# k2kobayashi/crank

Measured on AMD Instinct MI355X. Metric: train frames/sec, higher is better.
Workload: dtype bf16; 1 GPU; vqvae trainer step (all sub-updates), VCC2020-shaped synthetic 80-dim mlfb, 64 utterances x 500 frames per GPU, 14 speakers; trainer=vqvae, global_batch=64, batch_len=500, parallelism=dp1

## Files before the change

### crank_amd/_lib.py

```python
import ctypes
import os
from .config import cfg
from ctypes import c_char_p, c_double, c_float, c_int, c_longlong, c_ulonglong, c_void_p

_HERE = os.path.dirname(os.path.abspath(__file__))
LIB_PATH = cfg.lib_path or os.path.join(_HERE, "libcrank_hip.so")
_lib = None

ERRORS = {1: "invalid argument", 2: "HIP runtime error", 3: "unsupported shape/configuration"}


class NetDesc(ctypes.Structure):
    _fields_ = [
        ("kind", c_int), ("in_ch", c_int), ("out_ch", c_int), ("kernel_size", c_int), ("layers", c_int),
        ("stacks", c_int), ("res_ch", c_int), ("gate_ch", c_int), ("skip_ch", c_int), ("aux_ch", c_int),
        ("conv_ch", c_int), ("causal", c_int), ("use_bias", c_int), ("slope", c_float), ("dropout", c_float),
    ]


COLLATE_MAX_STREAMS = 8


class CollateStream(ctypes.Structure):
    _fields_ = [("src", c_void_p), ("ld", c_int), ("col0", c_int), ("ncols", c_int), ("dst", c_void_p)]


class CollateDesc(ctypes.Structure):
    _fields_ = [
        ("n_streams", c_int), ("streams", CollateStream * COLLATE_MAX_STREAMS), ("utt_start", c_void_p),
        ("utt_spk", c_void_p), ("n_utt", c_int), ("n_spk", c_int), ("lcf0_raw", c_void_p),
        ("spk_lcf0_mean", c_void_p), ("spk_lcf0_std", c_void_p), ("raw", c_void_p), ("raw_start", c_void_p),
        ("fftl", c_int), ("hop", c_int),
    ]


ADAM_MAX_BLOCKS = 4


class AdamBlock(ctypes.Structure):
    _fields_ = [("params", c_void_p), ("grads", c_void_p), ("exp_avg", c_void_p), ("exp_avg_sq", c_void_p),
                ("n", c_longlong), ("lr_dev", c_void_p), ("step_dev", c_void_p)]


class StreamDesc(ctypes.Structure):
    _fields_ = [
        ("n_stacks", c_int), ("in_ch", c_int), ("out_ch", c_int), ("emb_dim", c_int * 3), ("emb_size", c_int * 3),
        ("cb_off", c_longlong * 3), ("enc_base", c_longlong * 3), ("dec_base", c_longlong * 3), ("causal", c_int),
        ("enc_f0", c_int), ("dec_f0", c_int), ("spk_dim", c_int), ("spk_onehot", c_int), ("n_spk", c_int),
        ("spk_off", c_longlong),
    ]


class F0StreamRound(ctypes.Structure):
    _fields_ = [("ids", c_void_p), ("utt", c_void_p), ("range", c_void_p), ("chan_bf", c_void_p), ("chan", c_void_p),
                ("n_ready", c_int), ("total_samples", c_longlong), ("total_channels", c_longlong),
                ("total_frames", c_longlong), ("total_events", c_longlong)]


P, I, LL, ULL, F, D = c_void_p, c_int, c_longlong, c_ulonglong, c_float, c_double

SIGNATURES = {
    "crk_net_create": (P, [ctypes.POINTER(NetDesc)]),
    "crk_net_destroy": (None, [P]),
    "crk_net_param_count": (LL, [P]),
    "crk_net_conv_count": (I, [P]),
    "crk_net_conv_info": (I, [P, I, ctypes.POINTER(c_longlong)]),
    "crk_net_saved_bytes": (LL, [P, I, I]),
    "crk_net_reserve": (I, [P, I, I]),
    "crk_net_scratch_bytes": (LL, [P, I, I]),
    "crk_debug_alloc_count": (LL, []),
    "crk_debug_net_paths": (I, [P, I, I]),
    "crk_debug_net_partials": (LL, [P, I, I, P, LL, P]),
    "crk_seed_next": (I, [P, P, P]),
    "crk_nets_wnorm_bwd": (I, [I, P, P]),
    "crk_nets_prepare": (I, [I, P, P, ULL, P, P]),
    "crk_nets_prepare_models": (I, [I, P, P, P, I, P, P]),
    "crk_net_forward": (I, [P, P, ULL, P, I, P, I, P, I, P, I, I, I, ULL, P]),
    "crk_net_backward": (I, [P, P, ULL, P, P, I, P, I, P, I, P, I, F, P, I, P, I, I, I, ULL, P]),
    "crk_net_backward_scaled": (I, [P, P, ULL, P, P, I, P, I, P, I, P, I, F, P, I, P, I, I, I, ULL, P, P, P]),
    "crk_net_embed_grad_supported": (I, [P, I, I, I]),
    "crk_net_backward_embed": (I, [P, P, ULL, P, P, I, P, I, P, I, P, I, F, P, I, I, I, ULL, P, LL, I, I, I, P, P]),
    "crk_vq_forward": (I, [P, I, P, I, I, I, P, P, I, P, I, P]),
    "crk_vq_forward_fused": (I, [P, I, P, I, P, I, P, I, I, I, P, P, I, P, I, P, P, P, P, P]),
    "crk_vq_image_bytes": (LL, [I, I]),
    "crk_vq_image_build_multi": (I, [I, P, P, I, P, P]),
    "crk_vq_ema_scratch_bytes": (LL, [I, I, I]),
    "crk_vq_ema_stats": (I, [P, I, P, I, I, I, P, P, P, P]),
    "crk_vq_ema_apply": (I, [P, P, P, P, P, I, I, D, D, P]),
    "crk_vq_ema_partial": (I, [P, I, P, I, I, I, P, P]),
    "crk_vq_ema_reduce_multi": (I, [I, P, P, P, P, P, P, P]),
    "crk_vq_ema_apply_multi": (I, [I, P, P, P, P, P, P, P, D, D, P]),
    "crk_vq_ema_partial_multi": (I, [I, P, P, P, P, P, P, P, P]),
    "crk_vq_ema_reduce_size_multi": (I, [I, P, P, P, P, P, P, P, D, D, P]),
    "crk_vq_ema_blend_multi": (I, [I, P, P, P, P, P, P, D, P]),
    "crk_vq_ema_blend_image_multi": (I, [I, P, P, P, P, P, P, D, P, P]),
    "crk_stft_loss_multi_fwd": (I, [P, I, P, I, I, I, I, I, P, P, P, P, F, P, P, P]),
    "crk_stft_loss_multi_fwd_grad": (I, [P, I, P, I, I, I, I, I, P, P, P, P, F, P, P, I, P, P]),
    "crk_stft_loss_multi_bwd": (I, [P, I, P, I, I, I, I, I, P, P, P, P, F, P, P, I, P]),
    "crk_loss_scratch_floats": (I, []),
    "crk_masked_loss_fwd": (I, [P, I, P, I, F, P, LL, I, I, P, P, P]),
    "crk_masked_loss_bwd": (I, [P, I, P, I, F, P, LL, I, I, P, P, P, I, P, I, P]),
    "crk_masked_loss_both_fwd": (I, [P, I, P, I, P, LL, I, P, P, P]),
    "crk_weighted_sum": (I, [I, P, P, F, P, P]),
    "crk_weighted_sum_bwd": (I, [I, P, P, P, P]),
    "crk_recon_supported": (I, [I, I, P, P, P]),
    "crk_stft_twiddle_floats": (LL, [I, I]),
    "crk_stft_twiddles": (I, [I, I, P, P, P]),
    "crk_recon_grad_floats": (LL, [I, I, I, I, P, P]),
    "crk_recon_loss_fwd": (I, [P, I, P, I, P, I, I, I, I, P, P, P, P, F, P, P, P, P]),
    "crk_recon_loss_bwd": (I, [P, I, P, I, P, I, I, I, I, P, P, P, P, P, P, P, P, P, I, P]),
    "crk_masked_loss_bwd_acc": (I, [P, I, P, I, F, P, LL, I, I, P, P, P, I, P, I, P, I, P, P]),
    "crk_vq_commit_bwd": (I, [P, I, P, I, P, LL, I, P, P, P, I, P, I, P, I, P, I, P, I, P]),
    "crk_ce_fwd": (I, [P, I, P, LL, I, I, P, P, P, P]),
    "crk_ce_bwd": (I, [P, LL, I, P, P, P, P]),
    "crk_stft_loss_fwd": (I, [P, I, P, I, I, I, I, I, I, I, P, F, F, I, P, P, P]),
    "crk_stft_loss_bwd": (I, [P, I, P, I, I, I, I, I, I, I, P, F, F, P, P, I, P]),
    "crk_adam_step": (I, [P, P, P, P, LL, P, P, F, F, F, I, P]),
    "crk_adam_step_multi": (I, [I, ctypes.POINTER(AdamBlock), F, F, F, I, P]),
    "crk_radam_step": (I, [P, P, P, P, LL, P, P, D, D, D, I, P]),
    "crk_lamb_step": (I, [P, P, P, P, P, P, I, P, I, P, P, P, P, D, D, D, I, P]),
    "crk_lamb_tile": (I, []),
    "crk_concat_embed": (I, [P, I, I, P, I, I, P, I, P, LL, P, I, P]),
    "crk_embed_bwd_scratch_floats": (LL, [LL, I, I]),
    "crk_embed_bwd": (I, [P, I, I, I, P, LL, I, P, P, P]),
    "crk_concat_embed_run": (I, [P, I, I, P, I, I, P, I, P, LL, LL, P, I, P]),
# ... 154 lines not shown
```

### crank_amd/csrc/conv_kernels.h

```cpp
#pragma once
#include <vector>

#include "runtime.h"

#define CRK_TM 128

enum { MODE_PLAIN = 0, MODE_RESFWD = 1, MODE_BWDA = 2 };

struct ConvP {
  const float* xa; int lda; int cinA; float scaleA;
  const float* xb; int ldb; int cinB; float scaleB;
  int act_in; float slope;
  float drop_p; unsigned long long drop_seed;
  const unsigned long long* drop_seed_ptr;
  int cin, cin_pad;
  const float* xc; int ldc; int cinC; int cinC_pad;
  const uint16_t* w_hi; const uint16_t* w_lo;
  const uint16_t* wc_hi; const uint16_t* wc_lo;
  const uint16_t* w2_hi; const uint16_t* w2_lo;
  const float* bias; const float* bias2a; const float* bias2b;
  int cout, cout_pad, ktaps, dil, off0;
  int B, T, tiles_per_utt;
  float* y; int ldy; int accumulate; int act_out; float out_scale;
  const float* dmask; int ldm; int dmask_act;
// ... 164 lines not shown
  int rec;
  int dbg;
};
struct StackWLayer {
  long long pt_conv, pb_conv, pt_os, pb_os, pt_aux;
  int dil, off0;
};
struct StackWP {
  const uint16_t *xb_hi, *xb_lo, *zb_hi, *zb_lo, *cb_hi, *cb_lo;
  const uint16_t *gb_hi, *gb_lo, *dxb_hi, *dxb_lo, *dsb_hi, *dsb_lo;
  const StackWLayer* layers;
  float* partials;
  int B, T, L, ktaps, aux_ch, aux_pad, cpg, G;
  int rec_g;
  float* usums; int nseg;
};
int stack_wgrad_supported(int ktaps, int max_dil, int aux_ch);
int launch_stack_wgrad(const StackWP& p, bool precise, hipStream_t s);
struct CondEmbedP {
  const float* usums; int nseg, cpg;
  const uint16_t *whi, *wlo;
  const StackBLayer* layers;
  const long long* idx; long long run;
  int B, T, L, c0, E, n_rows;
  float* dtable;
};
int launch_cond_embed_bwd(const CondEmbedP& p, hipStream_t s);
int stack_bwd_plan(StackBP& p, bool precise);
int stack2_bwd_plan(StackBP& p);
int launch_stack2_bwd(const StackBP& p, hipStream_t s);
int stack_bwd_waves(bool precise);
int launch_stack_bwd(const StackBP& p, bool precise, hipStream_t s);
int stack_fwd_plan(StackP& p, bool precise);
int launch_stack_fwd(const StackP& p, bool precise, hipStream_t s);
int stack2_fwd_plan(StackP& p);
int launch_stack2_fwd(const StackP& p, hipStream_t s);
int stack2x_fwd_plan(StackP& p);
int launch_stack2x_fwd(const StackP& p, hipStream_t s);
void conv_fill_lds(ConvP& p, int mode, bool precise);
int launch_conv(const ConvP& p, int mode, bool precise, hipStream_t s);
int wgrad_expand(const WgradP& job, bool precise, std::vector<WgradP>& out);
int launch_wgrad_table(const WgradP* d_jobs, const std::vector<WgradP>& h_jobs, int B, int T, int max_groups, bool precise,
                       hipStream_t s);
#define CRK_MAX_NETS 8
struct NetRef {
  const ConvEntry* ents; const float* params; float* grads; const float* partials; float* norms;
  uint16_t *whi, *wlo;
  int n_ents, first;
};
#define CRK_MAX_BUMPS 4
struct NetRefs { NetRef r[CRK_MAX_NETS]; int n; float* bump[CRK_MAX_BUMPS]; int n_bump; };
int launch_weight_prep_multi(const NetRefs& R, int total_entries, int nmax, hipStream_t s);
int launch_step_bump(float* const* steps, int n, hipStream_t s);
int launch_wnorm_bwd_multi(const NetRefs& R, int total_entries, hipStream_t s);
int launch_weight_prep(const ConvEntry* d_entries, int n_entries, int nmax, const float* params, uint16_t* wprep_hi,
                       uint16_t* wprep_lo, float* norms, hipStream_t s);
int launch_wnorm_bwd(const ConvEntry* d_entries, int n_entries, const float* params, float* grads,
                     const float* partials, const float* norms, hipStream_t s);
int conv_kernels_init();
```

### crank_amd/csrc/conv_kernels.hip

```cpp
#include "conv_kernels.h"

__device__ __forceinline__ int cd_row(int r, int half) { return (r & 3) + 8 * (r >> 2) + 4 * half; }

__device__ __forceinline__ float load_src(const ConvP& p, long n, int c) {
  float v;
  if (c < p.cinA) {
    v = p.xa ? p.xa[n * p.lda + c] * p.scaleA : 0.f;
  } else {
    v = p.xb ? p.xb[n * p.ldb + (c - p.cinA)] * p.scaleB : 0.f;
  }
  v = apply_act(v, p.act_in, p.slope);
  if (p.drop_p > 0.f) v *= dropout_scale(crk_seed(p.drop_seed, p.drop_seed_ptr), (unsigned long long)n * p.cin + c, p.drop_p);
  return v;
}

template <bool PRECISE>
__device__ __forceinline__ void store4(unsigned char* hi, unsigned char* lo, const float v[4]) {
  *reinterpret_cast<uint2*>(hi) = make_uint2(pack_bf2(v[0], v[1]), pack_bf2(v[2], v[3]));
  if (PRECISE) {
    float r[4];
#pragma unroll
    for (int j = 0; j < 4; j++) r[j] = v[j] - bf2f(f2bf(v[j]));
    *reinterpret_cast<uint2*>(lo) = make_uint2(pack_bf2(r[0], r[1]), pack_bf2(r[2], r[3]));
  }
// ... 609 lines not shown
}
template <int BAND>
__global__ __launch_bounds__(256) void weight_prep_multi_kernel(const NetRefs R) {
  extern __shared__ unsigned wp_ws[];
  const NetRef& q = R.r[net_of_block(R, blockIdx.x)];
  const ConvEntry e = q.ents[blockIdx.x - q.first];
  if (blockIdx.x == 0 && blockIdx.y == 0) {
#pragma unroll
    for (int i = 0; i < CRK_MAX_BUMPS; i++)
      if (i < R.n_bump && (int)threadIdx.x == i) R.bump[i][0] += 1.f;
  }
  weight_prep_band<BAND>(e, blockIdx.y, q.params, q.whi, q.wlo, q.norms, wp_ws);
}
struct StepBumps { float* p[CRK_MAX_BUMPS]; };
__global__ void step_bump_kernel(const StepBumps b) {
#pragma unroll
  for (int i = 0; i < CRK_MAX_BUMPS; i++)
    if ((int)threadIdx.x == i) b.p[i][0] += 1.f;
}
int launch_step_bump(float* const* steps, int n, hipStream_t s) {
  if (n < 1 || n > CRK_MAX_BUMPS) return CRK_ERR_ARG;
  StepBumps b;
  for (int i = 0; i < CRK_MAX_BUMPS; i++) b.p[i] = steps[i < n ? i : 0];
  hipLaunchKernelGGL(step_bump_kernel, dim3(1), dim3(n), 0, s, b);
  CRK_CHECK_LAUNCH();
  return CRK_OK;
}
int launch_weight_prep_multi(const NetRefs& R, int total_entries, int nmax, hipStream_t s) {
  const size_t lds = (size_t)WP_BAND * nmax * 4;
  if (lds > 160 * 1024) return CRK_ERR_UNSUPPORTED;
  if (total_entries <= 16) {
    if (lds / 2 > 64 * 1024) CRK_RAISE_LDS_ONCE(160 * 1024, weight_prep_multi_kernel<8>)
    hipLaunchKernelGGL(weight_prep_multi_kernel<8>, dim3(total_entries, 128 / 8), dim3(256), lds / 2, s, R);
    CRK_CHECK_LAUNCH();
    return CRK_OK;
  }
  if (lds > 64 * 1024) CRK_RAISE_LDS_ONCE(160 * 1024, weight_prep_multi_kernel<WP_BAND>)
  hipLaunchKernelGGL(weight_prep_multi_kernel<WP_BAND>, dim3(total_entries, 128 / WP_BAND), dim3(256), lds, s, R);
  CRK_CHECK_LAUNCH();
  return CRK_OK;
}

int launch_weight_prep(const ConvEntry* d_entries, int n_entries, int nmax, const float* params, uint16_t* wprep_hi,
                       uint16_t* wprep_lo, float* norms, hipStream_t s) {
  const size_t lds = (size_t)WP_BAND * nmax * 4;
  if (lds > 160 * 1024) return CRK_ERR_UNSUPPORTED;
  if (lds > 64 * 1024) CRK_RAISE_LDS_ONCE(160 * 1024, weight_prep_kernel)
  dim3 grid(n_entries, 128 / WP_BAND), block(256);
  hipLaunchKernelGGL(weight_prep_kernel, grid, block, lds, s, d_entries, params, wprep_hi, wprep_lo, norms);
  CRK_CHECK_LAUNCH();
  return CRK_OK;
}

#ifndef WN_RB
#define WN_RB 8
#endif
#ifndef WN_IF
#define WN_IF 16
#endif
template <int RB> struct WnormShared { float dw[RB][128 * 8]; };
template <int RB, int IF>
__device__ __forceinline__ void wnorm_bwd_body(const ConvEntry& e, int band, const float* params, float* grads,
                                               const float* partials, const float* norms, WnormShared<RB>& sh) {
  const int co0 = band * RB;
  if (co0 >= e.cout) return;
  const int nrow = e.cout - co0 < RB ? e.cout - co0 : RB;
  const int G = e.pt_groups, k = e.k, cin = e.cin, cx = e.pt_cx;
  const int n = cin * k;
  const int tid = threadIdx.x;
  const long long gstride = (long long)e.pt_taps * e.pt_rows * e.pt_cx;
  const long long tstride = (long long)e.pt_rows * e.pt_cx;
  const float* base = partials + e.pt_off + (long long)(e.pt_row0 + co0) * cx;
  const int r = tid >> 5, l32 = tid & 31;
  const bool on = r < nrow;
  const int co = co0 + r;
  const float* __restrict__ v = params + e.off_v + (long long)co * n;
  float* __restrict__ gv = grads + e.off_v + (long long)co * n;
  constexpr int WN_PV = (128 * 8) / 32;
  float vr[WN_PV], go[WN_PV];
#pragma unroll
  for (int q = 0; q < WN_PV; q++) {
    const int i = l32 + 32 * q;
    const bool ok = on && i < n;
    vr[q] = ok ? v[i] : 0.f;
    go[q] = ok ? gv[i] : 0.f;
  }
  float sb = 0.f;
  if (on && e.off_b >= 0)
    for (int g = l32; g < e.pt_groups; g += 32) sb += partials[e.pb_off + (long long)g * e.pt_rows + e.pt_row0 + co];
  const float nrm = on ? norms[e.norm_off + co] : 1.f;
  const float gval = on ? params[e.off_g + co] : 0.f;
  const float g_old = (on && l32 == 0) ? grads[e.off_g + co] : 0.f;
  const float b_old = (on && l32 == 0 && e.off_b >= 0) ? grads[e.off_b + co] : 0.f;
  const int run = nrow * cx;
  if ((cx & 3) == 0 && ((((uintptr_t)base) & 15) == 0) && ((gstride | tstride) & 3) == 0) {
    const int run4 = run >> 2;
    for (int it = tid; it < k * run4; it += 256) {
      const int tap = it / run4, i4 = it - tap * run4;
      const float* src = base + tap * tstride + 4 * i4;
      f32x4 s4 = {0.f, 0.f, 0.f, 0.f};
      int g = 0;
      for (; g + IF <= G; g += IF) {
        f32x4 t[IF];
#pragma unroll
        for (int u = 0; u < IF; u++) t[u] = *reinterpret_cast<const f32x4*>(src + (long long)(g + u) * gstride);
#pragma unroll
        for (int u = 0; u < IF; u++) s4 += t[u];
      }
      if (IF > 16) {
        for (; g + 16 <= G; g += 16) {
          f32x4 t[16];
#pragma unroll
// ... 13 lines not shown
      const int r = (4 * i4) / cx, ci = 4 * i4 - r * cx;
#pragma unroll
      for (int j = 0; j < 4; j++) sh.dw[r][(ci + j) * k + tap] = s4[j] * e.pt_scale;
    }
  } else {
    for (int tap = 0; tap < k; tap++) {
      for (int i = tid; i < run; i += 256) {
        const float* src = base + tap * tstride + i;
        float sv = 0.f;
        int g = 0;
        for (; g + 8 <= G; g += 8) {
          float t[8];
#pragma unroll
          for (int u = 0; u < 8; u++) t[u] = src[(long long)(g + u) * gstride];
#pragma unroll
          for (int u = 0; u < 8; u++) sv += t[u];
        }
        for (; g < G; g++) sv += src[(long long)g * gstride];
        const int r = i / cx, ci = i - r * cx;
        sh.dw[r][ci * k + tap] = sv * e.pt_scale;
      }
    }
  }
  __syncthreads();
  float dot = 0.f;
#pragma unroll
  for (int q = 0; q < WN_PV; q++) {
    const int i = l32 + 32 * q;
    if (on && i < n) dot += sh.dw[r][i] * vr[q];
  }
#pragma unroll
  for (int o = 16; o > 0; o >>= 1) { dot += __shfl_xor(dot, o, 64); sb += __shfl_xor(sb, o, 64); }
  if (on) {
    const float inv = 1.f / nrm;
    if (l32 == 0) {
      grads[e.off_g + co] = g_old + dot * inv;
      if (e.off_b >= 0) grads[e.off_b + co] = b_old + sb * e.pt_scale;
    }
    const float c1 = gval * inv, c2 = dot * inv * inv;
#pragma unroll
    for (int q = 0; q < WN_PV; q++) {
      const int i = l32 + 32 * q;
      if (i < n) gv[i] = go[q] + c1 * (sh.dw[r][i] - c2 * vr[q]);
    }
  }
}

__global__ __launch_bounds__(256) void wnorm_bwd_kernel(const ConvEntry* ents, const float* params, float* grads,
                                                       const float* partials, const float* norms) {
  __shared__ WnormShared<WN_RB> sh;
  const ConvEntry e = ents[blockIdx.x];
  wnorm_bwd_body<WN_RB, WN_IF>(e, blockIdx.y, params, grads, partials, norms, sh);
}
template <int RB, int IF>
__global__ __launch_bounds__(256) void wnorm_bwd_multi_kernel(const NetRefs R) {
  __shared__ WnormShared<RB> sh;
  const NetRef& q = R.r[net_of_block(R, blockIdx.x)];
  const ConvEntry e = q.ents[blockIdx.x - q.first];
  wnorm_bwd_body<RB, IF>(e, blockIdx.y, q.params, q.grads, q.partials, q.norms, sh);
}
#define WN_SMALL_ENTRIES 16
int launch_wnorm_bwd_multi(const NetRefs& R, int total_entries, hipStream_t s) {
  if (total_entries <= WN_SMALL_ENTRIES) hipLaunchKernelGGL((wnorm_bwd_multi_kernel<2, 32>), dim3(total_entries, 128 / 2), dim3(256), 0, s, R);
  else hipLaunchKernelGGL((wnorm_bwd_multi_kernel<WN_RB, WN_IF>), dim3(total_entries, 128 / WN_RB), dim3(256), 0, s, R);
  CRK_CHECK_LAUNCH();
  return CRK_OK;
}


int launch_wnorm_bwd(const ConvEntry* d_entries, int n_entries, const float* params, float* grads,
                     const float* partials, const float* norms, hipStream_t s) {
  dim3 grid(n_entries, 128 / WN_RB), block(256);
  hipLaunchKernelGGL(wnorm_bwd_kernel, grid, block, 0, s, d_entries, params, grads, partials, norms);
  CRK_CHECK_LAUNCH();
  return CRK_OK;
}
```

### crank_amd/csrc/net.hip

```cpp
#include <math.h>
#include <stdlib.h>
#include <string.h>

#include <deque>
#include <vector>

#include "conv_kernels.h"

#include "../../include/crank_hip.h"

enum { ROLE_FIRST = 0, ROLE_CONV = 1, ROLE_AUX = 2, ROLE_OUT = 3, ROLE_SKIP = 4, ROLE_LAST1 = 5, ROLE_LAST2 = 6, ROLE_PLAIN = 7 };

struct ConvMeta {
  int role, layer, dilation;
};

static bool g_may_alloc = false;
static long long g_net_allocs = 0;
static hipError_t net_malloc_(void** p, size_t bytes) {
  if (!g_may_alloc) return hipErrorInvalidValue;
  g_net_allocs++;
  return hipMalloc(p, bytes);
}
#define NET_MALLOC(pp, bytes) net_malloc_(reinterpret_cast<void**>(pp), (bytes))
struct AllocScope {
  bool was;
  AllocScope() : was(g_may_alloc) { g_may_alloc = true; }
  ~AllocScope() { g_may_alloc = was; }
};
static int not_reserved(const char* what) {
  fprintf(stderr, "[crank_hip] %s: this batch shape needs device buffers / tables the handle does not hold - call "
                  "crk_net_reserve(net, B, T) once per batch shape, outside the step (the compute entry points never allocate)\n", what);
  return CRK_ERR_ARG;
}

#define PS_MAXL 16
struct PsTables { PsLayer t[4][PS_MAXL]; int L[4]; PwLayer w[PS_MAXL]; int nw; int max_wa, max_wb, max_tiles; double wflops_per_frame; };
struct ShapeNeed { long long need_s, need_p; int Gs, Gg, cpg, cpg_s, nseg; };
struct Route {
  bool fused;
  bool gen_split;
  bool x3f;
  bool disc_split;
  bool usums;
  unsigned char ps_fwd;
  unsigned char ps_fwd_x3f;
  unsigned char ps_bwd[2];
  bool fold_fwd;
  bool blocks_s2;
  bool fold_bwd_fs;
};
enum { CHAIN_PS = 0, CHAIN_PS2 = 1, CHAIN_PS2X = 2 };
struct Shape {
  int B, T;
  ShapeNeed q;
  Route route[2];
  bool pair_fused;
  std::vector<ConvEntry> abs;
  ConvEntry* d_ents = nullptr;
  PsTables ps;
  PsLayer* d_ps = nullptr;
  PwLayer* d_pw = nullptr;
  StackWLayer* d_wlayers = nullptr;
};

struct Net {
  crk_net_desc d;
  std::vector<ConvEntry> ents;
  std::vector<ConvMeta> meta;
  ConvEntry* d_ents = nullptr;
  long long n_params = 0;
  long long wprep_elems = 0, norm_elems = 0;
  uint16_t *whi = nullptr, *wlo = nullptr;
  float* norms = nullptr;
  unsigned long long prepared_version = ~0ull;
  const float* prepared_params = nullptr;
  const Shape* wn_shape = nullptr; const float* wn_params = nullptr; float* wn_grads = nullptr;
  const Shape* pw_shape = nullptr; PwP pw_params;
  float* partials = nullptr; long long partial_cap = 0;
  float* scratch = nullptr; long long scratch_cap = 0;
  long long pt_floats_stack = 0, pt_floats_gen = 0;
  int L = 0;
  int idx_first = -1, idx_last1 = -1, idx_last2 = -1;
  std::vector<int> idx_conv, idx_aux, idx_out, idx_skip, idx_plain;
  StackLayer* d_layers = nullptr;
  StackBLayer* d_blayers = nullptr;
  std::deque<Shape> shapes;
  std::vector<void*> retired;
  struct FwdTag { const float* saved; int B, T; unsigned char mode; bool x3f, fused; };
  FwdTag fwd_tags[32]; int fwd_tag_next = 0; int fwd_tag_count = 0;
  std::vector<WgradP> jobs;
  WgradP* d_jobs = nullptr;
  WgradP* h_slot[4] = {nullptr, nullptr, nullptr, nullptr};
  hipEvent_t slot_ev[4];
  int slot_next = 0;
};

static int pad16(int c) { return round_up(c, 16); }
static int pad32(int c) { return round_up(c, 32); }

static void add_conv(Net* n, int role, int layer, int cout, int cin, int k, int dil, bool bias) {
  ConvEntry e;
  memset(&e, 0, sizeof(e));
  e.cout = cout; e.cin = cin; e.k = k;
  if (bias) { e.off_b = n->n_params; n->n_params += cout; } else e.off_b = -1;
  e.off_g = n->n_params; n->n_params += cout;
  e.off_v = n->n_params; n->n_params += (long long)cout * cin * k;
  e.norm_off = n->norm_elems; n->norm_elems += cout;
  e.bw_off = -1; e.fr_off = -1; e.fr_mode = 0; e.bfr_off = -1; e.bfr_mode = 0;
  n->ents.push_back(e);
  n->meta.push_back({role, layer, dil});
}
// ... 118 lines not shown
        }
        break;
      }
    }
  }
  bool ok = true;
  ok = ok && NET_MALLOC(&n->whi, sizeof(uint16_t) * n->wprep_elems) == hipSuccess;
  ok = ok && NET_MALLOC(&n->wlo, sizeof(uint16_t) * n->wprep_elems) == hipSuccess;
  ok = ok && NET_MALLOC(&n->norms, sizeof(float) * n->norm_elems) == hipSuccess;
  ok = ok && hipMemset(n->whi, 0, sizeof(uint16_t) * n->wprep_elems) == hipSuccess;
  ok = ok && hipMemset(n->wlo, 0, sizeof(uint16_t) * n->wprep_elems) == hipSuccess;
  if (ok && (d.kind == 0 || d.kind == 1)) {
    std::vector<StackLayer> lt(n->L);
    for (int l = 0; l < n->L; l++) {
      const ConvEntry& ec = n->ents[n->idx_conv[l]];
      const ConvEntry& eo = n->ents[n->idx_out[l]];
      const ConvEntry& es = n->ents[n->idx_skip[l]];
      StackLayer& y = lt[l];
      y.w_conv = ec.fw_off; y.w_os = eo.fw_off;
      y.w_aux = d.aux_ch > 0 ? n->ents[n->idx_aux[l]].fw_off : 0;
      y.f_conv = ec.fr_off; y.f_os = eo.fr_off;
      y.f_aux = d.aux_ch > 0 ? n->ents[n->idx_aux[l]].fr_off : -1;
      y.b_conv = ec.off_b; y.b_out = eo.off_b; y.b_skip = es.off_b;
      y.dil = n->meta[n->idx_conv[l]].dilation;
      y.off0 = d.causal ? -(ec.k - 1) * y.dil : -((ec.k - 1) / 2) * y.dil;
    }
    ok = upload(&n->d_layers, lt.data(), n->L) == CRK_OK;
    std::vector<StackBLayer> bt(n->L);
    for (int l = 0; l < n->L; l++) {
      const ConvEntry& ec = n->ents[n->idx_conv[l]];
      const ConvEntry& eo = n->ents[n->idx_out[l]];
      StackBLayer& y = bt[l];
      y.w_conv = ec.bw_off; y.w_os = eo.bw_off;
      y.w_aux = d.aux_ch > 0 ? n->ents[n->idx_aux[l]].bw_off : 0;
      y.dil = n->meta[n->idx_conv[l]].dilation;
      const int off0 = d.causal ? -(ec.k - 1) * y.dil : -((ec.k - 1) / 2) * y.dil;
      y.off0 = -off0 - (ec.k - 1) * y.dil;
      y.f_conv = ec.bfr_off; y.f_os = eo.bfr_off;
      y.f_aux = d.aux_ch > 0 ? n->ents[n->idx_aux[l]].bfr_off : -1;
    }
    ok = ok && upload(&n->d_blayers, bt.data(), n->L) == CRK_OK;
  }
  ok = ok && upload(&n->d_ents, n->ents.data(), n->ents.size()) == CRK_OK;
  if (!ok) {
    fprintf(stderr, "[crank_hip] net_create: device allocation failed\n");
    delete n;
    return nullptr;
  }
  return n;
}

static void free_shape(Shape& r) {
  (void)hipFree(r.d_ents); (void)hipFree(r.d_ps); (void)hipFree(r.d_pw); (void)hipFree(r.d_wlayers);
}
extern "C" void crk_net_destroy(void* h) {
  Net* n = (Net*)h;
  if (!n) return;
  for (Shape& r : n->shapes) free_shape(r);
  for (void* q : n->retired) (void)hipFree(q);
  (void)hipFree(n->whi); (void)hipFree(n->wlo); (void)hipFree(n->norms); (void)hipFree(n->d_ents);
  for (int k = 0; k < 4; k++) if (n->h_slot[k]) { (void)hipHostFree(n->h_slot[k]); (void)hipEventDestroy(n->slot_ev[k]); }
  (void)hipFree(n->partials); (void)hipFree(n->scratch); (void)hipFree(n->d_jobs); (void)hipFree(n->d_layers); (void)hipFree(n->d_blayers);
  delete n;
}

extern "C" long long crk_net_param_count(void* h) { return ((Net*)h)->n_params; }
extern "C" int crk_net_conv_count(void* h) { return (int)((Net*)h)->ents.size(); }
extern "C" int crk_net_conv_info(void* h, int i, long long* out) {
  Net* n = (Net*)h;
  if (i < 0 || i >= (int)n->ents.size()) return CRK_ERR_ARG;
  const ConvEntry& e = n->ents[i];
  out[0] = e.cout; out[1] = e.cin; out[2] = e.k; out[3] = e.off_b; out[4] = e.off_g; out[5] = e.off_v;
  out[6] = n->meta[i].dilation; out[7] = n->meta[i].role; out[8] = n->meta[i].layer;
  return CRK_OK;
}

static int stack_aux_pad(const Net* n) { return n->d.aux_ch > 0 ? n->ents[n->idx_aux[0]].fw_kp : 16; }
struct GatedF32 {
  long long x, ta, sb, z, skip, h1, saved_total;
  long long ds, dh1, dx, dg, scratch_total;
};
static GatedF32 gated_f32(const Net* n, long long N) {
  const long long P = N * 64, LP = n->L * P;
  return {0, LP, 2 * LP, 3 * LP, 4 * LP, 4 * LP + P, 4 * LP + 2 * P, 0, P, 2 * P, 3 * P + LP, 3 * P + 3 * LP};
}
static long long saved_f32_floats(const Net* n, long long N) {
  return n->d.kind == 2 ? (long long)(n->L - 1) * N * n->d.conv_ch : gated_f32(n, N).saved_total;
}
static long long plain_planes_w(const Net* n) {
  long long w = 0;
  for (int i = 0; i < n->L; i++) w += n->ents[n->idx_plain[i]].fw_kp;
  return w;
}
static long long plain_gplanes_w(const Net* n) {
  long long w = 0;
  for (int i = 0; i < n->L; i++) w += n->ents[n->idx_plain[i]].bw_kp;
  return w;
}
struct GatedB16 {
  long long xb_hi, xb_lo, zb_hi, zb_lo, tb_hi, tb_lo, sg_hi, sg_lo, cb_hi, cb_lo, f_hi, f_lo, head_hi, head_lo, total;
};
static long long ts_plane_stride(long long N) { return ((N + 31) & ~31ll) * 64; }
static GatedB16 gated_b16(const Net* n, long long N) {
  GatedB16 g;
  const long long P = N * 64, LP = (long long)n->L * P, ca = N * stack_aux_pad(n), kf = N * n->ents[n->idx_first].fw_kp;
  const long long LPt = (long long)n->L * ts_plane_stride(N);
// ... 506 lines not shown
  }
  return fwd_layers(n, k, a);
}

static int stack_cpg(const Net* n, int B, int T) {
  const int ncpu = (T + 63) / 64;
  const int groups = crk_sw().wg_groups;
  const int gsz = (B + groups - 1) / groups;
  int cpg = gsz * ncpu;
  if (crk_sw().wg_fill && n->d.kind != 2 && n->L > 0 && 256 / n->L > groups) {
    const int fill = 256 / n->L;
    const int c = (B * ncpu + fill - 1) / fill;
    if (c >= 1 && c < cpg) cpg = c;
  }
  return cpg < 1 ? 1 : cpg;
}
static int stack_groups(const Net* n, int B, int T) {
  const int total = B * ((T + 63) / 64), cpg = stack_cpg(n, B, T);
  return (total + cpg - 1) / cpg;
}

static int usum_nseg(const Net* n, int B, int T) {
  const int ncpu = (T + 63) / 64;
  return (stack_cpg(n, B, T) + 2 * ncpu - 2) / ncpu;
}
static long long usum_floats(const Net* n, int B, int T) {
  if (n->d.kind == 2 || n->d.aux_ch <= 0) return 0;
  return (long long)stack_groups(n, B, T) * usum_nseg(n, B, T) * n->L * 128;
}
static long long usum_off(const Net* n, long long N) { return gated_f32(n, N).scratch_total + (gated_s16(n, N).total + 1) / 2; }
static ShapeNeed shape_need(const Net* n, int B, int T) {
  ShapeNeed q;
  const long long N = (long long)B * T;
  const long long cw = n->d.conv_ch > n->d.out_ch ? n->d.conv_ch : n->d.out_ch;
  q.need_s = n->d.kind == 2 ? (long long)n->L * N * cw + N * plain_gplanes_w(n)
                            : usum_off(n, N) + usum_floats(n, B, T);
  q.Gs = stack_groups(n, B, T); q.cpg_s = stack_cpg(n, B, T); q.nseg = usum_nseg(n, B, T);
  const int total_chunks = B * ((T + 63) / 64);
  const int groups = (n->d.kind == 2 && n->ents.size() <= 4) ? 64 : 32;
  q.cpg = (total_chunks + groups - 1) / groups;
  if (crk_sw().wg_cpg > 0) q.cpg = crk_sw().wg_cpg;
  q.Gg = (total_chunks + q.cpg - 1) / q.cpg;
  q.need_p = n->pt_floats_stack * q.Gs + n->pt_floats_gen * q.Gg;
  return q;
}
static int grow(Net* n, float** buf, long long* cap, long long need) {
  if (need <= *cap) return CRK_OK;
  if (*buf) n->retired.push_back(*buf);
  *buf = nullptr; *cap = 0;
  if (NET_MALLOC(buf, need * 4) != hipSuccess) return CRK_ERR_HIP;
  *cap = need;
  return CRK_OK;
}
static int build_shape(Net* n, Shape& r) {
  const crk_net_desc& d = n->d;
  r.abs = n->ents;
  for (auto& e : r.abs) {
    const bool stack = e.pt_groups != 0;
    const long long base = stack ? 0 : n->pt_floats_stack * r.q.Gs;
    const int G = stack ? r.q.Gs : r.q.Gg;
    e.pt_off = base + e.pt_off * G; e.pb_off = base + e.pb_off * G; e.pt_groups = G;
  }
  RUN(upload(&r.d_ents, r.abs.data(), r.abs.size()));
  if (n->L <= PS_MAXL) {
    ps_build(n, (long long)r.B * r.T, r.abs.data(), r.ps);
    RUN(upload(&r.d_ps, &r.ps.t[0][0], 4 * PS_MAXL));
    RUN(upload(&r.d_pw, r.ps.w, PS_MAXL));
  }
  if (d.kind != 2) {
    std::vector<StackWLayer> wt(n->L);
    for (int l = 0; l < n->L; l++) {
      const ConvEntry& ec = n->ents[n->idx_conv[l]];
      const ConvEntry& eo = n->ents[n->idx_out[l]];
      const ConvEntry& ac = r.abs[n->idx_conv[l]];
      const ConvEntry& ao = r.abs[n->idx_out[l]];
      StackWLayer& y = wt[l];
      y.pt_conv = ac.pt_off; y.pb_conv = ec.off_b >= 0 ? ac.pb_off : -1;
      y.pt_os = ao.pt_off; y.pb_os = eo.off_b >= 0 ? ao.pb_off : -1;
      y.pt_aux = d.aux_ch > 0 ? r.abs[n->idx_aux[l]].pt_off : 0;
      y.dil = n->meta[n->idx_conv[l]].dilation;
      y.off0 = fwd_off0(n, ec.k, y.dil);
    }
    RUN(upload(&r.d_wlayers, wt.data(), wt.size()));
  }
  return CRK_OK;
}
extern "C" int crk_net_reserve(void* h, int B, int T) {
  Net* n = (Net*)h;
  if (!n || B <= 0 || T <= 0) return CRK_ERR_ARG;
  if (find_shape(n, B, T)) return CRK_OK;
  AllocScope may_allocate;
  Shape r{};
  r.B = B; r.T = T; r.q = shape_need(n, B, T);
  r.route[0] = route_of(n, B, T, false);
  r.route[1] = route_of(n, B, T, true);
  r.pair_fused = routes_pair_fused(r.route);
  RUN(grow(n, &n->scratch, &n->scratch_cap, r.q.need_s));
  RUN(grow(n, &n->partials, &n->partial_cap, r.q.need_p));
  if (!n->d_jobs && NET_MALLOC(&n->d_jobs, sizeof(WgradP) * 256) != hipSuccess) return CRK_ERR_HIP;
  const int rc = build_shape(n, r);
  if (rc != CRK_OK) {
    free_shape(r);
    return rc;
  }
  n->shapes.push_back(r);
  return CRK_OK;
}
extern "C" long long crk_net_scratch_bytes(void* h, int B, int T) {
  Net* n = (Net*)h;
  if (!n || B <= 0 || T <= 0) return -1;
  const ShapeNeed q = shape_need(n, B, T);
  return (q.need_s + q.need_p) * 4;
}
extern "C" long long crk_debug_alloc_count(void) { return g_net_allocs; }
long long crk_count_alloc_(void) { return ++g_net_allocs; }
extern "C" int crk_debug_net_paths(void* h, int B, int T) {
// ... 392 lines not shown
                   .s = (hipStream_t)stream};
  return net_backward_impl(h, version, flags, seed, a);
}

__global__ void seed_next_kernel(unsigned long long* state, unsigned long long* out) {
  unsigned long long z = (*state += 0x9E3779B97F4A7C15ull);
  z = (z ^ (z >> 30)) * 0xBF58476D1CE4E5B9ull;
  z = (z ^ (z >> 27)) * 0x94D049BB133111EBull;
  *out = (z ^ (z >> 31)) & 0x3fffffffffffffffull;
}
extern "C" int crk_seed_next(unsigned long long* state, unsigned long long* out, void* stream) {
  if (!state || !out) return CRK_ERR_ARG;
  hipLaunchKernelGGL(seed_next_kernel, dim3(1), dim3(1), 0, (hipStream_t)stream, state, out);
  CRK_CHECK_LAUNCH();
  return CRK_OK;
}

static int flush_plain_wgrads(int n_nets, void* const* nets, hipStream_t s) {
  PwMP M; memset(&M, 0, sizeof(M));
  int blocks = 0, max_wa = 0, max_wb = 0, max_tiles = 0, pending = 0;
  double flops = 0.0, bytes = 0.0;
  Net* only = nullptr;
  for (int i = 0; i < n_nets; i++) {
    Net* n = (Net*)nets[i];
    if (!n) return CRK_ERR_ARG;
    if (n->pw_shape) { pending++; only = n; }
  }
  if (pending == 1 && only->d.kind == 2) return flush_pending_plain_wgrad(only, s);
  for (int i = 0; i < n_nets; i++) {
    Net* n = (Net*)nets[i];
    const Shape* r = n->pw_shape;
    if (!r) continue;
    if (M.n == CRK_MAX_NETS_PW) { RUN(flush_pending_plain_wgrad(n, s)); continue; }
    const PsTables& Tb = r->ps;
    M.q[M.n] = n->pw_params;
    M.first[M.n] = blocks;
    blocks += Tb.nw * n->pw_params.G;
    if (Tb.max_wa > max_wa) max_wa = Tb.max_wa;
    if (Tb.max_wb > max_wb) max_wb = Tb.max_wb;
    if (Tb.max_tiles > max_tiles) max_tiles = Tb.max_tiles;
    flops += Tb.wflops_per_frame * r->B * r->T;
    bytes += 2.0 * (Tb.max_wa + Tb.max_wb) * (double)r->B * r->T * Tb.nw;
    M.n++;
    n->pw_shape = nullptr;
  }
  M.first[M.n] = blocks;
  if (M.n > 0) RUN(launch_pstack_wgrad_multi(M, blocks, max_wa, max_wb, max_tiles, flops, bytes, s));
  return CRK_OK;
}
extern "C" int crk_nets_wnorm_bwd(int n_nets, void* const* nets, void* stream) {
  if (n_nets < 0 || (n_nets > 0 && !nets)) return CRK_ERR_ARG;
  hipStream_t s = (hipStream_t)stream;
  RUN(flush_plain_wgrads(n_nets, nets, s));
  NetRefs R; memset(&R, 0, sizeof(R));
  int total = 0;
  for (int i = 0; i < n_nets; i++) {
    Net* n = (Net*)nets[i];
    if (!n) return CRK_ERR_ARG;
    if (!n->wn_shape) continue;
    if (R.n == CRK_MAX_NETS) {
      RUN(flush_pending_wnorm(n, s));
      continue;
    }
    NetRef& q = R.r[R.n++];
    q.ents = n->wn_shape->d_ents; q.n_ents = (int)n->ents.size(); q.first = total;
    q.params = n->wn_params; q.grads = n->wn_grads; q.partials = n->partials; q.norms = n->norms;
    total += q.n_ents;
    n->wn_shape = nullptr;
  }
  if (R.n == 0) return CRK_OK;
  return launch_wnorm_bwd_multi(R, total, s);
}

extern "C" int crk_nets_prepare_models(int n_nets, void* const* nets, const float* const* params,
                                       const unsigned long long* versions, int n_bumps, float* const* bump_steps,
                                       void* stream) {
  if (n_nets < 0 || (n_nets > 0 && (!nets || !params || !versions))) return CRK_ERR_ARG;
  if (n_bumps < 0 || n_bumps > CRK_MAX_BUMPS || (n_bumps > 0 && !bump_steps)) return CRK_ERR_ARG;
  for (int i = 0; i < n_bumps; i++) if (!bump_steps[i]) return CRK_ERR_ARG;
  for (int i = 0; i < n_nets; i++) if (!nets[i] || !params[i]) return CRK_ERR_ARG;
  hipStream_t s = (hipStream_t)stream;
  NetRefs R; memset(&R, 0, sizeof(R));
  int total = 0, nmax = 1;
  for (int i = 0; i < n_nets; i++) {
    Net* n = (Net*)nets[i];
    if (n->prepared_version == versions[i] && n->prepared_params == params[i]) continue;
    if (net_nmax(n) > nmax) nmax = net_nmax(n);
    if (R.n == CRK_MAX_NETS) { RUN(ensure_prepared(n, params[i], versions[i], s)); continue; }
    NetRef& q = R.r[R.n++];
    q.ents = n->d_ents; q.n_ents = (int)n->ents.size(); q.first = total;
    q.params = params[i]; q.whi = n->whi; q.wlo = n->wlo; q.norms = n->norms;
    total += q.n_ents;
    n->prepared_version = versions[i]; n->prepared_params = params[i];
  }
  if (R.n == 0) return n_bumps ? launch_step_bump(bump_steps, n_bumps, s) : CRK_OK;
  for (int i = 0; i < n_bumps; i++) R.bump[i] = bump_steps[i];
  R.n_bump = n_bumps;
  return launch_weight_prep_multi(R, total, nmax, s);
}
extern "C" int crk_nets_prepare(int n_nets, void* const* nets, const float* const* params, unsigned long long version,
                                float* bump_step, void* stream) {
  if (n_nets < 0 || (n_nets > 0 && (!nets || !params))) return CRK_ERR_ARG;
  const std::vector<unsigned long long> versions((size_t)n_nets + 1, version);
  return crk_nets_prepare_models(n_nets, nets, params, versions.data(), bump_step ? 1 : 0, &bump_step, stream);
}
```

### include/crank_hip.h

```cpp
#ifndef CRANK_HIP_H
#define CRANK_HIP_H
#ifdef __cplusplus
extern "C" {
#endif

#define CRK_OK 0
#define CRK_ERR_ARG 1
#define CRK_ERR_HIP 2
#define CRK_ERR_UNSUPPORTED 3

#define CRK_FLAG_PRECISE 1
#define CRK_FLAG_NO_PARAM_GRAD 2
#define CRK_FLAG_NO_SAVE 4
#define CRK_FLAG_DEFER_WNORM 8

#define CRK_FLAG_SEED_ON_DEVICE 16
#define CRK_FLAG_FWD_PRECISE 32
#define CRK_FLAG_BWD_PLAIN 64

typedef struct crk_net_desc {
  int kind;
  int in_ch, out_ch, kernel_size, layers, stacks;
  int res_ch, gate_ch, skip_ch, aux_ch;
  int conv_ch;
// ... 334 lines not shown
               const long long* sample_offsets, int n_utts, long long total_frames, long long total_samples, int n_iter,
               int clip, double* y, void* workspace, long long workspace_bytes, void* stream);
int crk_gl_stft(void* gl, const double* x, const long long* frame_offsets, const long long* sample_offsets, int n_utts,
                long long total_frames, long long total_samples, double* spec, void* stream);
int crk_gl_istft(void* gl, const double* spec, const long long* frame_offsets, const long long* sample_offsets, int n_utts,
                 long long total_frames, long long total_samples, double* y, void* workspace, long long workspace_bytes,
                 void* stream);

typedef struct crk_stream_desc {
  int n_stacks, in_ch, out_ch;
  int emb_dim[3], emb_size[3];
  long long cb_off[3], enc_base[3], dec_base[3];
  int causal, enc_f0, dec_f0;
  int spk_dim, spk_onehot, n_spk;
  long long spk_off;
} crk_stream_desc;
int crk_stream_create(const crk_stream_desc* desc, void* const* enc_nets, void* const* dec_nets, void** handle);
void crk_stream_destroy(void* st);
int crk_stream_reserve(void* st, int S, int C_max);
long long crk_stream_state_bytes(void* st, int S);
int crk_stream_prepare(void* st, const float* params, unsigned long long version, void* stream);
int crk_stream_reset(void* st, const int* stream_ids, int n, void* stream);
int crk_stream_push(void* st, const float* x, int ldx, const float* dec_cond, int ldd, const float* enc_cond, int lde,
                    const long long* spk, const int* n_valid, int S, int C, float* decoded, long long* const* qidx,
                    float* const* encoded, void* stream);

int crk_lstream_create(const crk_stream_desc* desc, void* const* enc_nets, void* const* dec_nets, void** handle);
void crk_lstream_destroy(void* st);
int crk_lstream_lookahead(void* st);
int crk_lstream_reserve(void* st, int S, int C_max);
long long crk_lstream_state_bytes(void* st, int S);
int crk_lstream_prepare(void* st, const float* params, unsigned long long version, void* stream);
int crk_lstream_reset(void* st, const int* stream_ids, int n, void* stream);
int crk_lstream_push(void* st, const float* x, int ldx, const float* dec_cond, int ldd, const float* enc_cond, int lde,
                     const long long* spk, const int* n_valid, const int* end, int S, int C, int rows_out, float* decoded,
                     long long* const* qidx, float* const* encoded, int* n_out, int* first, void* stream);

int crk_join_create(int n_streams, int width_a, int width_b, int max_in_a, int max_in_b, int cap_a, int cap_b, void** handle);
void crk_join_destroy(void* st);
long long crk_join_state_bytes(void* st);
int crk_join_max_frames(void* st);
int crk_join_reset(void* st, const int* stream_ids, int n, void* stream);
int crk_join_push(void* st, const float* a, int lda, const int* n_a, const float* b, int ldb, const int* n_b, const int* end,
                  int S, float* out_a, int ldoa, float* out_b, int ldob, int C_out, int* n_out, int* first_out,
                  int* n_dropped, void* stream);
int crk_join_status(void* st, int* flags, void* stream);
int crk_feat_renorm(const float* x, int ldx, const float* scale, const float* mean, const float* vmean, const float* vscale,
                    const int* n_valid, int S, int C, int width, float* out, int ldo, void* stream);

long long crk_debug_alloc_count(void);

int crk_debug_net_paths(void* net, int B, int T);
long long crk_debug_net_partials(void* net, int B, int T, float* out, long long cap, void* stream);

const char* crk_version(void);

#ifdef __cplusplus
}
#endif
#endif
```

Before: 21.68 million frames/s.

## Replace weight-norm backward with band-list streaming kernel over precomputed row bands

Weight-norm backward previously launched a 2D grid of (conv entry x fixed 128/RB bands), so many blocks handled empty rows when cout was small. It now builds a host-side list holding only the real row bands per conv, sorted by partial-reduction size so the largest go first. It uploads the list once per shape and launches one block per band. The new kernel streams the per-group partial sums with double-buffered vector loads (float4 when aligned) and reduces across groups, cutting idle blocks and improving load throughput. Small nets keep a separate small-band path, and a debug query for the band list is added.

```diff
diff --git a/crank_amd/_lib.py b/crank_amd/_lib.py
--- a/crank_amd/_lib.py
+++ b/crank_amd/_lib.py
@@ -71,6 +71,7 @@
     "crk_debug_alloc_count": (LL, []),
     "crk_debug_net_paths": (I, [P, I, I]),
     "crk_debug_net_partials": (LL, [P, I, I, P, LL, P]),
+    "crk_debug_net_wnorm_bands": (LL, [P, I, I, P, LL]),
     "crk_seed_next": (I, [P, P, P]),
     "crk_nets_wnorm_bwd": (I, [I, P, P]),
     "crk_nets_prepare": (I, [I, P, P, ULL, P, P]),
diff --git a/crank_amd/csrc/conv_kernels.h b/crank_amd/csrc/conv_kernels.h
--- a/crank_amd/csrc/conv_kernels.h
+++ b/crank_amd/csrc/conv_kernels.h
@@ -240,7 +240,26 @@
 struct NetRefs { NetRef r[CRK_MAX_NETS]; int n; float* bump[CRK_MAX_BUMPS]; int n_bump; };
 int launch_weight_prep_multi(const NetRefs& R, int total_entries, int nmax, hipStream_t s);
 int launch_step_bump(float* const* steps, int n, hipStream_t s);
-int launch_wnorm_bwd_multi(const NetRefs& R, int total_entries, hipStream_t s);
+struct WnBand {
+  long long src;
+  long long gstride, tstride;
+  long long pb;
+  long long off_v, off_g, off_b;
+  long long norm;
+  int k, cin, cx, rows, groups, pb_stride;
+  float scale;
+  int conv;
+};
+#define WN_BAND 8
+#define WN_SMALL_ENTRIES 16
+#define WN_BAND_SMALL 2
+struct WnRef {
+  const WnBand* bands; const float* params; float* grads; const float* partials; const float* norms;
+  int first;
+};
+struct WnRefs { WnRef r[CRK_MAX_NETS]; int n; };
+int launch_wnorm_bwd_multi(const WnRefs& R, int total_bands, hipStream_t s);
+int launch_wnorm_bwd_small(const NetRefs& R, int total_entries, hipStream_t s);
 int launch_weight_prep(const ConvEntry* d_entries, int n_entries, int nmax, const float* params, uint16_t* wprep_hi,
                        uint16_t* wprep_lo, float* norms, hipStream_t s);
 int launch_wnorm_bwd(const ConvEntry* d_entries, int n_entries, const float* params, float* grads,
diff --git a/crank_amd/csrc/conv_kernels.hip b/crank_amd/csrc/conv_kernels.hip
--- a/crank_amd/csrc/conv_kernels.hip
+++ b/crank_amd/csrc/conv_kernels.hip
@@ -685,12 +685,8 @@
   return CRK_OK;
 }
 
-#ifndef WN_RB
 #define WN_RB 8
-#endif
-#ifndef WN_IF
 #define WN_IF 16
-#endif
 template <int RB> struct WnormShared { float dw[RB][128 * 8]; };
 template <int RB, int IF>
 __device__ __forceinline__ void wnorm_bwd_body(const ConvEntry& e, int band, const float* params, float* grads,
@@ -810,21 +806,17 @@
   const ConvEntry e = ents[blockIdx.x];
   wnorm_bwd_body<WN_RB, WN_IF>(e, blockIdx.y, params, grads, partials, norms, sh);
 }
-template <int RB, int IF>
-__global__ __launch_bounds__(256) void wnorm_bwd_multi_kernel(const NetRefs R) {
-  __shared__ WnormShared<RB> sh;
+__global__ __launch_bounds__(256) void wnorm_bwd_small_kernel(const NetRefs R) {
+  __shared__ WnormShared<WN_BAND_SMALL> sh;
   const NetRef& q = R.r[net_of_block(R, blockIdx.x)];
   const ConvEntry e = q.ents[blockIdx.x - q.first];
-  wnorm_bwd_body<RB, IF>(e, blockIdx.y, q.params, q.grads, q.partials, q.norms, sh);
-}
-#define WN_SMALL_ENTRIES 16
-int launch_wnorm_bwd_multi(const NetRefs& R, int total_entries, hipStream_t s) {
-  if (total_entries <= WN_SMALL_ENTRIES) hipLaunchKernelGGL((wnorm_bwd_multi_kernel<2, 32>), dim3(total_entries, 128 / 2), dim3(256), 0, s, R);
-  else hipLaunchKernelGGL((wnorm_bwd_multi_kernel<WN_RB, WN_IF>), dim3(total_entries, 128 / WN_RB), dim3(256), 0, s, R);
+  wnorm_bwd_body<WN_BAND_SMALL, 32>(e, blockIdx.y, q.params, q.grads, q.partials, q.norms, sh);
+}
+int launch_wnorm_bwd_small(const NetRefs& R, int total_entries, hipStream_t s) {
+  hipLaunchKernelGGL(wnorm_bwd_small_kernel, dim3(total_entries, 128 / WN_BAND_SMALL), dim3(256), 0, s, R);
   CRK_CHECK_LAUNCH();
   return CRK_OK;
 }
-
 
 int launch_wnorm_bwd(const ConvEntry* d_entries, int n_entries, const float* params, float* grads,
                      const float* partials, const float* norms, hipStream_t s) {
diff --git a/crank_amd/csrc/net.hip b/crank_amd/csrc/net.hip
--- a/crank_amd/csrc/net.hip
+++ b/crank_amd/csrc/net.hip
@@ -2,6 +2,7 @@
 #include <stdlib.h>
 #include <string.h>
 
+#include <algorithm>
 #include <deque>
 #include <vector>
 
@@ -58,6 +59,8 @@
   bool pair_fused;
   std::vector<ConvEntry> abs;
   ConvEntry* d_ents = nullptr;
+  std::vector<WnBand> wn;
+  WnBand* d_wn = nullptr;
   PsTables ps;
   PsLayer* d_ps = nullptr;
   PwLayer* d_pw = nullptr;
@@ -282,6 +285,7 @@
 
 static void free_shape(Shape& r) {
   (void)hipFree(r.d_ents); (void)hipFree(r.d_ps); (void)hipFree(r.d_pw); (void)hipFree(r.d_wlayers);
+  (void)hipFree(r.d_wn);
 }
 extern "C" void crk_net_destroy(void* h) {
   Net* n = (Net*)h;
@@ -894,6 +898,34 @@
   *cap = need;
   return CRK_OK;
 }
+static int wnorm_band_list(const std::vector<ConvEntry>& ents, int rb, std::vector<WnBand>& out) {
+  out.clear();
+  for (size_t ei = 0; ei < ents.size(); ei++) {
+    const ConvEntry& e = ents[ei];
+    if (e.cout > 128 || e.pt_cx < e.cin || e.pt_cx * e.k > 128 * 8 || e.pt_groups < 1) return CRK_ERR_UNSUPPORTED;
+    for (int co0 = 0; co0 < e.cout; co0 += rb) {
+      WnBand b;
+      memset(&b, 0, sizeof(b));
+      b.src = e.pt_off + (long long)(e.pt_row0 + co0) * e.pt_cx;
+      b.gstride = (long long)e.pt_taps * e.pt_rows * e.pt_cx;
+      b.tstride = (long long)e.pt_rows * e.pt_cx;
+      b.pb = e.pb_off + e.pt_row0 + co0;
+      b.off_v = e.off_v + (long long)co0 * e.cin * e.k;
+      b.off_g = e.off_g + co0;
+      b.off_b = e.off_b >= 0 ? e.off_b + co0 : -1;
+      b.norm = e.norm_off + co0;
+      b.k = e.k; b.cin = e.cin; b.cx = e.pt_cx;
+      b.rows = e.cout - co0 < rb ? e.cout - co0 : rb;
+      b.groups = e.pt_groups; b.pb_stride = e.pt_rows;
+      b.scale = e.pt_scale;
+      b.conv = (int)ei;
+      out.push_back(b);
+    }
+  }
+  auto bytes = [](const WnBand& b) { return 4ll * b.groups * b.k * b.rows * b.cx; };
+  std::stable_sort(out.begin(), out.end(), [&](const WnBand& a, const WnBand& b) { return bytes(a) > bytes(b); });
+  return CRK_OK;
+}
 static int build_shape(Net* n, Shape& r) {
   const crk_net_desc& d = n->d;
   r.abs = n->ents;
@@ -904,6 +936,8 @@
     e.pt_off = base + e.pt_off * G; e.pb_off = base + e.pb_off * G; e.pt_groups = G;
   }
   RUN(upload(&r.d_ents, r.abs.data(), r.abs.size()));
+  RUN(wnorm_band_list(r.abs, WN_BAND, r.wn));
+  if (!r.wn.empty()) RUN(upload(&r.d_wn, r.wn.data(), r.wn.size()));
   if (n->L <= PS_MAXL) {
     ps_build(n, (long long)r.B * r.T, r.abs.data(), r.ps);
     RUN(upload(&r.d_ps, &r.ps.t[0][0], 4 * PS_MAXL));
@@ -1402,8 +1436,9 @@
   if (n_nets < 0 || (n_nets > 0 && !nets)) return CRK_ERR_ARG;
   hipStream_t s = (hipStream_t)stream;
   RUN(flush_plain_wgrads(n_nets, nets, s));
-  NetRefs R; memset(&R, 0, sizeof(R));
-  int total = 0;
+  WnRefs R; memset(&R, 0, sizeof(R));
+  NetRefs S; memset(&S, 0, sizeof(S));
+  int bands = 0, convs = 0;
   for (int i = 0; i < n_nets; i++) {
     Net* n = (Net*)nets[i];
     if (!n) return CRK_ERR_ARG;
@@ -1412,14 +1447,33 @@
       RUN(flush_pending_wnorm(n, s));
       continue;
     }
-    NetRef& q = R.r[R.n++];
-    q.ents = n->wn_shape->d_ents; q.n_ents = (int)n->ents.size(); q.first = total;
-    q.params = n->wn_params; q.grads = n->wn_grads; q.partials = n->partials; q.norms = n->norms;
-    total += q.n_ents;
+    const Shape* r = n->wn_shape;
+    NetRef& p = S.r[S.n++];
+    p.ents = r->d_ents; p.n_ents = (int)n->ents.size(); p.first = convs;
+    WnRef& q = R.r[R.n++];
+    q.bands = r->d_wn; q.first = bands;
+    q.params = p.params = n->wn_params; q.grads = p.grads = n->wn_grads;
+    q.partials = p.partials = n->partials; q.norms = p.norms = n->norms;
+    bands += (int)r->wn.size(); convs += p.n_ents;
     n->wn_shape = nullptr;
   }
   if (R.n == 0) return CRK_OK;
-  return launch_wnorm_bwd_multi(R, total, s);
+  if (convs <= WN_SMALL_ENTRIES) return launch_wnorm_bwd_small(S, convs, s);
+  return launch_wnorm_bwd_multi(R, bands, s);
+}
+extern "C" long long crk_debug_net_wnorm_bands(void* h, int B, int T, long long* out, long long cap) {
+  Net* n = (Net*)h;
+  const Shape* r = n ? find_shape(n, B, T) : nullptr;
+  if (!r || cap < 0 || (cap > 0 && !out)) return -1;
+  const std::vector<WnBand>& L = r->wn;
+  for (long long i = 0; i < (long long)L.size() && i < cap; i++) {
+    const WnBand& b = L[i];
+    const ConvEntry& e = r->abs[b.conv];
+    out[6 * i + 0] = b.conv; out[6 * i + 1] = (b.off_g - e.off_g); out[6 * i + 2] = b.rows; out[6 * i + 3] = b.groups;
+    out[6 * i + 4] = 4ll * b.groups * b.k * b.rows * b.cx;
+    out[6 * i + 5] = (((long long)b.rows * b.cx | b.gstride | b.tstride | b.src) & 3) == 0;
+  }
+  return (long long)L.size();
 }
 
 extern "C" int crk_nets_prepare_models(int n_nets, void* const* nets, const float* const* params,
diff --git a/crank_amd/csrc/wnorm_kernels.hip b/crank_amd/csrc/wnorm_kernels.hip
--- /dev/null
+++ b/crank_amd/csrc/wnorm_kernels.hip
@@ -0,0 +1,165 @@
+#include "stack_common.h"
+
+template <int RB> struct WnStreamShared { float dw[RB][128 * 8]; };
+template <int V> struct WnPiece;
+template <> struct WnPiece<4> { typedef f32x4 T; };
+template <> struct WnPiece<1> { typedef float T; };
+
+__device__ __forceinline__ int wn_net_of_block(const WnRefs& R, int bx) {
+  int r = 0;
+  while (r + 1 < R.n && bx >= R.r[r + 1].first) r++;
+  return r;
+}
+
+template <int RB, int D, int V, class Mark>
+__device__ __forceinline__ void wn_stream_sum(const WnBand& w, const float* base, WnStreamShared<RB>& sh, Mark&& mark) {
+  typedef typename WnPiece<V>::T vec;
+  const int tid = threadIdx.x;
+  const int runv = (w.rows * w.cx) / V, total = w.k * runv;
+  const int G = w.groups, k = w.k, cx = w.cx;
+  const long long gstride = w.gstride;
+  const float scale = w.scale;
+  const int mine = tid < total ? (total - tid + 255) >> 8 : 0;
+  const int steps = __builtin_amdgcn_readfirstlane(mine) * ((G + D - 1) / D);
+  auto src_of = [&](int p) -> const float* {
+    int it = tid + (p << 8);
+    it = it < total ? it : total - 1;
+    const int tap = it / runv;
+    return base + tap * w.tstride + V * (it - tap * runv);
+  };
+  int ip = 0, ig = 0;
+  const float* isrc = src_of(0);
+  auto issue = [&](vec (&t)[D]) {
+#pragma unroll
+    for (int u = 0; u < D; u++) {
+      const int g = ig + u < G ? ig + u : G - 1;
+      t[u] = *reinterpret_cast<const vec*>(isrc + (long long)g * gstride);
+    }
+    ig += D;
+    if (ig >= G) { ig = 0; ip++; isrc = src_of(ip); }
+  };
+  int cp = 0, cg = 0;
+  vec s = {};
+  auto consume = [&](vec (&t)[D]) {
+#pragma unroll
+    for (int u = 0; u < D; u++) s = cg + u < G ? s + t[u] : s;
+    cg += D;
+    if (cg >= G) {
+      const int it = tid + (cp << 8);
+      if (it < total) {
+        const int tap = it / runv, e0 = V * (it - tap * runv);
+        int r = e0 / cx, ci = e0 - r * cx;
+#pragma unroll
+        for (int j = 0; j < V; j++) {
+          float sj;
+          if constexpr (V == 1) sj = s; else sj = s[j];
+          sh.dw[r][ci * k + tap] = sj * scale;
+          if (++ci == cx) { ci = 0; r++; }
+        }
+      }
+      s = vec{};
+      cg = 0; cp++;
+    }
+    mark();
+  };
+  vec a[D], b[D];
+  int j = 0;
+  if (steps > 0) issue(a);
+  for (; j + 2 < steps; j += 2) {
+    issue(b);
+    consume(a);
+    issue(a);
+    consume(b);
+  }
+  if (steps - j == 2) {
+    issue(b);
+    consume(a);
+    consume(b);
+  } else if (steps - j == 1) {
+    consume(a);
+  }
+}
+
+template <int RB, int D>
+__global__ __launch_bounds__(256) void wnorm_stream_kernel(const WnRefs R) {
+  __shared__ WnStreamShared<RB> sh;
+  SK_PROF_BEGIN()
+  const WnRef& q = R.r[wn_net_of_block(R, blockIdx.x)];
+  const WnBand w = q.bands[blockIdx.x - q.first];
+  const float* __restrict__ params = q.params;
+  float* __restrict__ grads = q.grads;
+  const float* __restrict__ partials = q.partials;
+  const int nrow = w.rows, G = w.groups;
+  const int n = w.cin * w.k;
+  const int tid = threadIdx.x;
+  const float* base = partials + w.src;
+  const int r = tid >> 5, l32 = tid & 31;
+  const bool on = r < nrow;
+  const float* __restrict__ v = params + w.off_v + (long long)r * n;
+  float* __restrict__ gv = grads + w.off_v + (long long)r * n;
+  constexpr int WN_PV = (128 * 8) / 32;
+  float vr[WN_PV], go[WN_PV];
+#pragma unroll
+  for (int p = 0; p < WN_PV; p++) {
+    const int i = l32 + 32 * p;
+    const bool ok = on && i < n;
+    vr[p] = ok ? v[i] : 0.f;
+    go[p] = ok ? gv[i] : 0.f;
+  }
+  const bool hb = on && w.off_b >= 0;
+  const float* __restrict__ pbp = partials + w.pb + r;
+  const float bp0 = (hb && l32 < G) ? pbp[(long long)l32 * w.pb_stride] : 0.f;
+  const float bp1 = (hb && l32 + 32 < G) ? pbp[(long long)(l32 + 32) * w.pb_stride] : 0.f;
+  const float nrm = on ? q.norms[w.norm + r] : 1.f;
+  const float gval = on ? params[w.off_g + r] : 0.f;
+  const float g_old = (on && l32 == 0) ? grads[w.off_g + r] : 0.f;
+  const float b_old = (on && l32 == 0 && w.off_b >= 0) ? grads[w.off_b + r] : 0.f;
+  SK_T(0)
+#ifdef SK_PROF
+  auto mark = [&]() { SK_T(1) pacc_[4] += 1; };
+#else
+  auto mark = []() {};
+#endif
+  if ((((nrow * w.cx) | (int)(w.gstride | w.tstride)) & 3) == 0 && ((((uintptr_t)base) & 15) == 0))
+    wn_stream_sum<RB, D, 4>(w, base, sh, mark);
+  else
+    wn_stream_sum<RB, D, 1>(w, base, sh, mark);
+  float sb = 0.f;
+  if (hb) {
+    if (l32 < G) sb += bp0;
+    if (l32 + 32 < G) sb += bp1;
+    for (int g = l32 + 64; g < G; g += 32) sb += pbp[(long long)g * w.pb_stride];
+  }
+  __syncthreads();
+  SK_T(2)
+  float dot = 0.f;
+#pragma unroll
+  for (int p = 0; p < WN_PV; p++) {
+    const int i = l32 + 32 * p;
+    if (on && i < n) dot += sh.dw[r][i] * vr[p];
+  }
+#pragma unroll
+  for (int o = 16; o > 0; o >>= 1) { dot += __shfl_xor(dot, o, 64); sb += __shfl_xor(sb, o, 64); }
+  if (on) {
+    const float inv = 1.f / nrm;
+    if (l32 == 0) {
+      grads[w.off_g + r] = g_old + dot * inv;
+      if (w.off_b >= 0) grads[w.off_b + r] = b_old + sb * w.scale;
+    }
+    const float c1 = gval * inv, c2 = dot * inv * inv;
+#pragma unroll
+    for (int p = 0; p < WN_PV; p++) {
+      const int i = l32 + 32 * p;
+      if (i < n) gv[i] = go[p] + c1 * (sh.dw[r][i] - c2 * vr[p]);
+    }
+  }
+  SK_T(3)
+  SK_PROF_END(5)
+}
+
+int launch_wnorm_bwd_multi(const WnRefs& R, int total_bands, hipStream_t s) {
+  if (total_bands <= 0) return CRK_OK;
+  hipLaunchKernelGGL((wnorm_stream_kernel<WN_BAND, 8>), dim3(total_bands), dim3(256), 0, s, R);
+  CRK_CHECK_LAUNCH();
+  return CRK_OK;
+}
diff --git a/include/crank_hip.h b/include/crank_hip.h
--- a/include/crank_hip.h
+++ b/include/crank_hip.h
@@ -410,6 +410,7 @@
 
 int crk_debug_net_paths(void* net, int B, int T);
 long long crk_debug_net_partials(void* net, int B, int T, float* out, long long cap, void* stream);
+long long crk_debug_net_wnorm_bands(void* net, int B, int T, long long* out, long long cap);
 
 const char* crk_version(void);
 
```

Measured after the change: 22.01 million frames/s, median of 4. +1.6%, better.
